# xaedes/ros_gpu_depthmap_fusion

Measured on AMD Instinct MI355X. Metric: Mpoints/s end-to-end depth→fused voxel grid @1/2/4/8 GPU; % HBM roofline, higher is better.
Workload: dtype f32; 1 GPU; C2: 640x480 u16 depth (dense frames), launch defaults (F=4 thr 0.3, crop/voxel -10..30/-20..20/-1..1.5, cells 0.1/0.1/0.12, voxelize average, lifetime 10); a step = a batch of 8 frames through one launch chain (every frame's points, voxel means and grid); cameras_per_gpu=1, steps=1630, warmup=5, prime=8, grid_cells=3360000, frames_in_flight=3, step_pmc_bytes=85523388, parallelism=single GPU

## Files before the change

### include/gdf.h

```cpp
#ifndef GDF_H_
#define GDF_H_

#include <stddef.h>
#include <stdint.h>

#ifdef __cplusplus
extern "C" {
#endif

#define GDF_VERSION_MAJOR 0
#define GDF_VERSION_MINOR 4

#define GDF_MAX_CAMERAS 16

enum gdf_status_code {
    GDF_OK = 0,
    GDF_ERR_ARG = -1,
    GDF_ERR_STATE = -2,
    GDF_ERR_HIP = -3,
    GDF_ERR_NOMEM = -4,
    GDF_ERR_CAPACITY = -5,
    GDF_ERR_TIME = -6,
    GDF_ERR_DEVICE = -7
};
// ... 129 lines not shown
    const float* points;
    const uint32_t* voxel_coords;
    uint32_t num_points;
    const float* voxelized;
    uint32_t num_voxelized;
    const uint8_t* occupancy;
    uint64_t num_cells;
} gdf_host_frame;
int gdf_download_frame(gdf_engine* engine, uint32_t what, gdf_host_frame* out);

int gdf_process_frame(gdf_engine* engine, const gdf_frame_params* params,
                      gdf_frame_result* out_result);

int gdf_get_graph_stats(gdf_engine* engine, uint64_t* captures, uint64_t* replays);
int gdf_last_sort_items(gdf_engine* engine, uint32_t* items, int* runs);

int gdf_mask_dilate(gdf_engine* engine, const uint32_t* in_mask_device, uint32_t* out_mask_device,
                    uint32_t width, uint32_t height, uint32_t filter_size, int as_written);
int gdf_transform_points(gdf_engine* engine, const float* in_points_device,
                         const uint32_t* mask_device, float* out_points_device, uint32_t num_items,
                         const float T[16]);

int gdf_next_frame_in_batch(gdf_engine* engine);
int gdf_get_batch_ranges(gdf_engine* engine, uint32_t* point_start, uint32_t* voxel_start,
                         uint32_t capacity, uint32_t* out_frames);
int gdf_download_batch_occupancy_grid(gdf_engine* engine, uint32_t frame, uint8_t* out,
                                      uint64_t capacity);

int gdf_export_occupancy_marks(gdf_engine* engine, uint32_t* device_bitmask, uint64_t words);
int gdf_import_occupancy_marks(gdf_engine* engine, const uint32_t* device_bitmasks,
// ... 85 lines not shown
```

### ros_gpu_depthmap_fusion_amd/csrc/gdf_device.hpp

```cpp
#pragma once

#include <hip/hip_runtime.h>
#include <stdint.h>

namespace gdf {

constexpr int kMaxCams = 16;
constexpr int kFrameThreads = 256;
constexpr int kArgCams = 8;
constexpr int kHalo = 8;
constexpr uint32_t kSegItems = 1024;
constexpr uint32_t kFusedPrefixSegs = 4096;
constexpr uint32_t kScanGroup = 64;
constexpr uint32_t kMaxScanGroups = 4096;
constexpr uint32_t kMaxGroupScanTiles = 65536;
constexpr uint32_t kSelSegs = 8;
constexpr uint32_t kSelThreads = 512;
constexpr int kSortThreads = 256;
constexpr int kSortGroup = 8;
constexpr int kHistReps = 16;
constexpr int kHistWords = kHistReps * 4 * 256;

__host__ __device__ constexpr uint32_t radix_passes(uint32_t bits) {
    return bits == 0 ? 1u : bits <= 25 ? (bits <= 9 ? 1u : (bits + 6) / 8) : (bits + 7) / 8;
}
__host__ __device__ constexpr bool radix_wide_last(uint32_t bits) {
    return bits >= 9 && bits <= 25 && bits % 8 == 1;
}
__host__ __device__ constexpr uint32_t radix_digit(uint32_t key, uint32_t p, uint32_t np) {
// ... 121 lines not shown
    uint32_t* grid_seq_out;
    uint32_t grid_seq;
    uint32_t nframes;
    uint32_t frame_shift;
    uint64_t mark_words;
    uint32_t* frame_pt_start;
    int32_t run_mode;
    uint32_t* wave_runs;
    uint32_t* run_keys;
    uint32_t* run_start;
    uint32_t* run_count;
    uint32_t* scan_total;
    uint32_t* run_total;
    uint32_t* grp_done;
    uint32_t* grp_tot;
    int32_t mask_packed;
    uint32_t nparts;
    uint64_t part_ncells;
    float4* part_pts;
    uint32_t* part_run_keys;
    uint32_t* part_run_starts;
    uint32_t* part_counts;
    uint32_t part_nseg;
    uint32_t seg_uniform;
    const Tuning* tune;
};
static_assert(sizeof(FrameArgs) <= 4096, "kernel arguments are limited to 4 KiB");

__device__ __forceinline__ float dot3(float ax, float ay, float az, float bx, float by, float bz) {
    return (ax * bx + ay * by) + az * bz;
// ... 52 lines not shown
```

### ros_gpu_depthmap_fusion_amd/csrc/gdf_engine.cpp

```cpp
#include <hip/hip_runtime.h>

#include <algorithm>
#include <cmath>
#include <cstdio>
#include <cstring>
#include <cstdlib>
#include <atomic>
#include <condition_variable>
#include <memory>
#include <mutex>
#include <string>
#include <thread>
#include <vector>

#include "gdf.h"
#include "gdf_kernels.hpp"

using namespace gdf;

namespace {
thread_local std::string g_last_error;
}

namespace gdf {
// ... 280 lines not shown
    DevBuf d_ka, d_kb, d_va, d_vb, d_sstatus, d_sgstatus, d_gstatus, d_ggstatus, d_vox;
    DevBuf d_gcnt, d_goff;
    DevBuf d_gfirst;
    DevBuf d_bigq, d_bigcnt;
    bool vox_valid = false;
    DevBuf d_markbits;
    uint32_t marks_gen = ~0u;
    uint32_t marks_frames = 0;
    DevBuf d_fstart, d_fvox;
    DevBuf d_snap_idx, d_snap_data, d_snap_cnt;
    bool snap_valid = false;
    uint32_t snap_blocks = 0, snap_frames = 0;
    DevBuf d_pcnt, d_poff;
    DevBuf d_xcnt, d_xoff, d_xrk, d_xrs;
    DevBuf d_grpdone, d_grptot;
    struct Pinned {
        void* p = nullptr;
        size_t bytes = 0;
        void* ensure(size_t need) {
            if (need <= bytes) return p;
            if (p) (void)hipHostFree(p);
            p = nullptr;
            bytes = 0;
            const size_t nb = std::max(need, bytes + bytes / 2);
            if (hipHostMalloc(&p, nb, hipHostMallocDefault) != hipSuccess) {
                p = nullptr;
                return nullptr;
            }
            bytes = nb;
            return p;
// ... 75 lines not shown
    PsBuf* collect = &psA;
    PsBuf* upload = &psB;

    std::vector<Cam> cams;
    uint32_t nframes = 1;
    uint32_t depth_total = 0;
    std::vector<CamDesc> halo;
    std::vector<Cam> halo_cams;
    std::vector<uint32_t> halo_tail;
    std::vector<CamTable> tables = std::vector<CamTable>(kMaxCams);
    std::vector<CamDesc> h_cams;
    uint32_t mask_blocks = 0;
    uint64_t index_end = 0;
    uint32_t last_sort_items = 0;
    bool last_sort_runs = false;
    uint32_t max_segw = 0;
    bool depth_uploaded = false;

    DevBuf d_new;
    uint32_t n_new = 0;
    std::vector<Hdr> new_hdrs;
    bool ps_filter_set = false;
    float ps_thr = 0.f;
    uint32_t ps_F = 0;

    DevBuf d_ring;
    uint64_t ring_cap = 0, ring_head = 0;
    std::vector<Hdr> hdrA, hdrB;
    uint32_t shard = 0, nshards = 1, shard_block = 1;
    uint64_t seq_counter = 0;
// ... 873 lines not shown
        q.d_runkeys.ensure((size_t)std::max<uint32_t>(q.n_total, 1) * 4);
        q.d_runstart.ensure(((size_t)q.n_total + 1) * 4);
        a.wave_runs = q.d_wruns.as<uint32_t>();
        a.run_keys = q.d_runkeys.as<uint32_t>();
        a.run_start = q.d_runstart.as<uint32_t>();
        a.run_count = q.d_misc.as<uint32_t>() + kRunCount;
        if (a.sel_tiles) a.run_total = q.d_misc.as<uint32_t>() + kRunTotal;
    }
    e->sl().runs_sel = a.run_mode && a.sel_tiles;
    a.vbits = e->sl().d_vbits.as<unsigned long long>();
    a.seg_counts = e->sl().d_tcounts.as<uint32_t>();
    a.seg_offsets = e->sl().d_toffsets.as<uint32_t>();
    a.fused_prefix = a.total_segs <= kFusedPrefixSegs ? 1 : 0;
    a.mask_packed = e->mask_packed ? 1 : 0;
    const uint32_t ngroups = (a.total_segs + kScanGroup - 1) / kScanGroup;
    if (!a.fused_prefix && e->group_scan && ngroups <= kMaxScanGroups) {
        Slot& q = e->sl();
        q.d_grpdone.ensure_zero((size_t)ngroups * 4, e->s());
        q.d_grptot.ensure((size_t)ngroups * 2 * 4);
        a.grp_done = q.d_grpdone.as<uint32_t>();
        a.grp_tot = q.d_grptot.as<uint32_t>();
    }
    {
        const uint32_t h = a.do_flying ? std::min<uint32_t>(a.F, kHalo) : 0u;
        const uint32_t cols = e->max_segw + 2 * h;
        a.band_rowb = ((cols * 2 + 15) / 16 + 1) * 16;
        a.band_lds = (2 * h + 1) * a.band_rowb + (kHalo + a.seg_threads * 2) * 4;
        a.hist_lds = (a.band_lds + 15) & ~15u;
        if (a.run_mode && a.key_hist) a.band_lds = a.hist_lds + 4 * 256 * 4;
    }
    if (e->debug) {
        e->sl().d_stage.ensure(std::max<size_t>({(size_t)e->sl().n_total, (size_t)e->index_end + sel, 1}));
        a.dbg = e->sl().d_stage.as<uint8_t>();
    }
    e->sl().dbg_count = e->sl().n_total;
    a.err = e->sl().d_misc.as<uint32_t>() + kErr;
    if (!e->halo_cams.empty() && a.do_flying && !e->cams.empty()) {
        for (size_t j = 0; j < e->halo_cams.size(); ++j) {
            const Cam* first = nullptr;
            for (const Cam& c : e->cams)
                if (c.frame == e->halo_cams[j].frame) { first = &c; break; }
            if (!first) continue;
            const uint64_t reach = (uint64_t)a.F * first->W + a.F;
            if (reach > e->halo_cams[j].n)
                fail(GDF_ERR_ARG, "halo camera shorter than F rows of the frame's first camera "
                                  "(reads would reach the camera before it)");
            if (e->halo_tail[j] < reach)
                fail(GDF_ERR_ARG, "halo depth map tail shorter than F rows + F pixels of the frame's first camera");
        }
    }
    a.nframes = e->nframes;
    a.frame_shift = e->nframes > 1 ? e->key_bits : 0u;
    a.mark_words = mark_words(e);
    e->sl().sel_frame = a.sel_tiles != 0;
    if (fused_voxel && compaction_marks && e->epart.nparts && e->emit_part && !a.sel_tiles &&
        a.total_segs && !e->debug) {
        FrameArgs t = a;
        t.run_mode = 1;
        t.key_hist = nullptr;
        t.fused_prefix = 0;
        t.grp_done = t.grp_tot = nullptr;
        if (emit_partition_kernels(t)) {
            Slot& q = e->sl();
            const uint32_t segs = std::max<uint32_t>(a.total_segs, 1);
            const uint32_t P = e->epart.nparts;
            q.d_tcounts.ensure((size_t)segs * 2 * P * 4);
            q.d_toffsets.ensure(seg_offsets_words(2 * P * segs) * 4);
            q.d_wruns.ensure((size_t)segs * 16 * 4);
            t.seg_counts = q.d_tcounts.as<uint32_t>();
            t.seg_offsets = q.d_toffsets.as<uint32_t>();
            t.wave_runs = q.d_wruns.as<uint32_t>();
            t.nparts = P;
            t.part_ncells = e->ncells;
            t.part_pts = reinterpret_cast<float4*>(e->epart.pts);
            t.part_run_keys = e->epart.run_keys;
            t.part_run_starts = e->epart.run_starts;
            t.part_counts = e->epart.counts;
            t.part_nseg = e->epart.nseg;
            a = t;
        }
    }
    e->sl().nframes = e->nframes;
    e->sl().snap_valid = false;
    if (e->nframes > 1) {
        e->sl().d_fstart.ensure((size_t)(e->nframes + 1) * 4);
        a.frame_pt_start = e->sl().d_fstart.as<uint32_t>();
    }
    return a;
}

void frame_launched(gdf_engine* e, bool fused_voxel, bool key_hist, bool runs = false) {
    e->sl().khist_pending = fused_voxel && key_hist;
    e->sl().runs_valid = fused_voxel && runs;
    e->sl().compacted = true;
    e->sl().coords_valid = fused_voxel;
    e->sl().marks_set = fused_voxel;
    e->sl().vox_valid = false;
}

void run_frame(gdf_engine* e, bool fused_voxel, bool compaction_marks = false) {
    e->sl().pf_valid = false;
    const FrameArgs a = frame_args(e, fused_voxel, compaction_marks);
// ... 1189 lines not shown
            e->last_sort_runs = runs;
            e->last_sort_items = runs ? e->sl().h_misc[e->sl().runs_sel ? kRunTotal : kRunCount]
                                      : res.num_points;
        }
        if (r) *r = res;
    });
}

int gdf_last_sort_items(gdf_engine* e, uint32_t* items, int* runs) {
    ENGINE_OR_FAIL(e);
    if (items) *items = e->last_sort_items;
    if (runs) *runs = e->last_sort_runs ? 1 : 0;
    return GDF_OK;
}

int gdf_mask_dilate(gdf_engine* e, const uint32_t* in, uint32_t* out, uint32_t W, uint32_t H,
                    uint32_t F, int as_written) {
    ENGINE_OR_FAIL(e);
    return guarded(e, [&] {
        if ((!in || !out) && (uint64_t)W * H) fail(GDF_ERR_ARG, "mask_dilate: null mask");
        if (in == out && (uint64_t)W * H) fail(GDF_ERR_ARG, "mask_dilate: in-place is not supported");
        if (F > kDilateMaxF) fail(GDF_ERR_ARG, "mask_dilate: filter size above 16");
        HIPCHK(launch_mask_dilate(in, out, W, H, F, as_written, e->s()));
    });
}

int gdf_transform_points(gdf_engine* e, const float* in, const uint32_t* mask, float* out,
                         uint32_t n, const float T[16]) {
    ENGINE_OR_FAIL(e);
    return guarded(e, [&] {
// ... 490 lines not shown
```

### ros_gpu_depthmap_fusion_amd/csrc/gdf_kernels.hip

```cpp
#include <atomic>
#include "gdf_kernels.hpp"

#if defined(__HIP_DEVICE_COMPILE__) && !defined(__gfx950__)
#error "gdf_kernels.hip targets gfx950 (CDNA4) only: its coherence hand-offs use gfx950 cache bits"
#endif
#include "gdf_voxsum.hpp"

#include <algorithm>

namespace gdf {

template <class T>
using gptr = __attribute__((address_space(1))) T*;
template <class T>
__device__ __forceinline__ gptr<T> G(T* p) {
    return (gptr<T>)p;
}

typedef float f4v __attribute__((ext_vector_type(4)));
__device__ __forceinline__ float4 gld4(const float4* p, uint64_t i) {
    const f4v v = ((gptr<const f4v>)p)[i];
    return make_float4(v.x, v.y, v.z, v.w);
}
__device__ __forceinline__ void gst4(float4* p, uint64_t i, const float4& w) {
// ... 686 lines not shown
__device__ __forceinline__ void group_partials_finish(const FrameArgs& a, uint32_t s,
                                                      const GroupPart& p, uint32_t* s_red) {
    const int lane = threadIdx.x & 63, wid = threadIdx.x >> 6;
    const uint32_t g = s / kScanGroup;
    const uint32_t ng = (a.total_segs + kScanGroup - 1) / kScanGroup;
    uint32_t sum = 0, rsum = 0;
#pragma unroll
    for (int q = 0; q < 4; ++q) {
        const bool in = threadIdx.x + (uint32_t)q * blockDim.x < g;
        sum += in ? p.v[q] : 0u;
        rsum += in ? p.w[q] : 0u;
    }
    for (uint32_t t = threadIdx.x + 4u * blockDim.x; t < g; t += blockDim.x) {
        sum += G(a.grp_tot)[t];
        if (a.run_mode) rsum += G(a.grp_tot)[ng + t];
    }
    for (int o = 32; o > 0; o >>= 1) {
        sum += __shfl_xor(sum, o, 64);
        rsum += __shfl_xor(rsum, o, 64);
    }
    if (lane == 0) {
        s_red[wid] = sum;
        s_red[16 + wid] = rsum;
    }
}

template <bool ROT45, uint32_t FT>
__global__ __launch_bounds__(1024) void k_mask(FrameArgs a) {
    __shared__ CamDesc s_cams[kMaxCams];
    __shared__ float s_yn[2 * kHalo + 1];
// ... 373 lines not shown
    uint32_t* s_hist = reinterpret_cast<uint32_t*>(reinterpret_cast<uint8_t*>(s_dyn) + a.hist_lds);
    const int lane = threadIdx.x & 63, wid = threadIdx.x >> 6;
    if (a.nparts)
        for (uint32_t j = threadIdx.x; j < 2u * NWORDS * kMaxParts; j += NT) (&s_pc[0][0][0])[j] = 0u;
    const uint32_t n = gridDim.x, q8 = n / 8, r8 = n % 8, xcd = blockIdx.x % 8;
    const uint32_t s = xcd * q8 + min(xcd, r8) + blockIdx.x / 8;
    uint32_t bits[PX], rkey[PX];
#pragma unroll
    for (int j = 0; j < PX; ++j) {
        bits[j] = 0u;
        rkey[j] = 0xFFFFFFFFu;
    }
    const uint32_t i = threadIdx.x;
    if (a.run_mode && a.key_hist)
        for (uint32_t j = threadIdx.x; j < radix_hist_span(a.npasses); j += NT) s_hist[j] = 0;
    {
        const gptr<const CamDesc> gcam = G(cam_table(a));
        SegGeo sg = seg_geo(gcam, a.ncams, s, a.seg_uniform);
        struct {
            const uint16_t* depth;
            const float *xn, *yn;
            uint32_t W, H;
        } c = {gcam[sg.k].depth, gcam[sg.k].xn, gcam[sg.k].yn, gcam[sg.k].W, gcam[sg.k].H};
#ifdef GDF_TRACE_GROUPS
        asm volatile("" ::"s"(c.depth), "s"(c.W));
        GDF_MSTAMP(1);
#endif
        const int h = 4;
        const uint32_t ca = sg.x0 >= (uint32_t)h ? sg.x0 - h : 0u;
        const uint32_t cb = min(c.W, sg.x0 + sg.len + h);
        const uint32_t nrows = 2 * h + 1;
        uint8_t* band = reinterpret_cast<uint8_t*>(s_dyn);
        float* s_xn = reinterpret_cast<float*>(band + (size_t)nrows * a.band_rowb) + kHalo;
        const bool wrap = sg.x0 == 0 && sg.y >= (uint32_t)h && c.W >= (uint32_t)h;
        typedef uint32_t u4v __attribute__((ext_vector_type(4)));
        const uintptr_t dbase = reinterpret_cast<uintptr_t>(c.depth);
        const uint32_t nch = a.band_rowb / 16;
        u4v v[QR][QC];
// ... 153 lines not shown
    __syncthreads();
#ifdef GDF_TRACE_GROUPS
    GDF_MSTAMP(5);
#endif
    if (wid == 0) {
        if (a.nparts) {
            if ((uint32_t)lane < 2u * a.nparts) {
                const uint32_t kind = lane / a.nparts, p = lane % a.nparts;
                uint32_t c = 0;
                for (int w = 0; w < NWORDS; ++w) c += s_pc[kind][w][p];
                G(a.seg_counts)[(size_t)lane * a.total_segs + s] = c;
            }
        } else if (lane == 0) {
            uint32_t tt = 0, r = 0;
            for (int w = 0; w < NWORDS; ++w) tt += s_cnt[w];
            publish_count(a.seg_counts + s, tt);
            if (a.run_mode) {
                for (int w = 0; w < NWORDS; ++w) r += s_rcnt[w];
                publish_count(a.seg_counts + a.total_segs + s, r);
            }
        }
    }
    if (a.run_mode && a.key_hist) {
        const gptr<uint32_t> rep = G(a.key_hist + (blockIdx.x % kHistReps) * 1024u);
        for (uint32_t j = threadIdx.x; j < radix_hist_span(a.npasses); j += NT)
            if (s_hist[j])
                __hip_atomic_fetch_add(rep + j, s_hist[j], __ATOMIC_RELAXED, __HIP_MEMORY_SCOPE_AGENT);
    }
    if (a.grid_seq_out && blockIdx.x == 0 && threadIdx.x == 0) *a.grid_seq_out = a.grid_seq;
    group_scan_tail(a, s);
#ifdef GDF_TRACE_GROUPS
    GDF_MSTAMP(6);
    if (threadIdx.x == 0 && blockIdx.x < kMaskTraceSlots) {
        unsigned long long* g = g_mtrace[blockIdx.x];
        g[0] = mw0;
        g[1] = wall_clock64();
        for (int k = 1; k < 7; ++k) g[k + 1] = mt[k] - mt[k - 1];
    }
#endif
}

template <int PX, int SEGW>
__global__ __launch_bounds__(SEGW / PX) void k_mask_px(FrameArgs a) {
    mask_px_body<PX, SEGW>(a);
}
// ... 416 lines not shown
        asm volatile("" : "+s"(vw[w]));
        any |= vw[w];
    }
    if (!__builtin_amdgcn_readfirstlane((uint32_t)(any | (any >> 32))) && s != nblk - 1) {
        if (!fps) return;
        const bool first_of_frame =
            s == seg0 && (k == 0 || !cams[k - 1].emit || cams[k - 1].frame != fr);
        if (!first_of_frame) return;
    }
    for (uint32_t j = threadIdx.x; j < (1u << kMarkCacheBits); j += NT) s_mark[j] = 0xFFFFFFFFu;
    const bool hist = a.key_hist && !a.run_mode;
    if (hist)
        for (uint32_t i = threadIdx.x; i < radix_hist_span(a.npasses); i += NT) s_hist[i] = 0;
    GroupPart gp{};
    if (!a.fused_prefix && a.grp_tot) gp = group_partials_issue(a, s);
    const uint32_t i = threadIdx.x;
    const uint32_t j = s - seg0;
    const uint32_t y = j / nchunk;
    const uint32_t x0 = (j - y * nchunk) * segw;
    const uint32_t len = min(segw, W - x0);
    uint64_t m[2];
    uint32_t dval[2] = {0u, 0u};
    float xnv[2] = {0.0f, 0.0f};
    uint16_t dl[2];
    float xl[2];
#pragma unroll
    for (int q = 0; q < 2; ++q) {
        m[q] = 0;
#pragma unroll
        for (int w = 0; w < NW; ++w)
// ... 3 lines not shown
        xl[q] = G(cxn)[x0 + ic];
    }
#pragma unroll
    for (int q = 0; q < 2; ++q) {
        const bool in = i + (uint32_t)NT * q < len;
        dval[q] = in ? dl[q] : 0u;
        xnv[q] = in ? xl[q] : 0.0f;
    }
    const float ynv = G(cyn)[y];
    uint32_t pc[NWORDS], rc[NWORDS];
#pragma unroll
    for (int w = 0; w < NWORDS; ++w) {
        pc[w] = (uint32_t)__popcll(vw[w]);
        rc[w] = 0u;
    }
    const uint32_t sbase = a.fused_prefix ? 0u : G(a.seg_offsets)[s];
    uint32_t rbase = 0;
    if (a.run_mode) {
        if (!a.fused_prefix)
            rbase = G(a.seg_offsets)[a.total_segs + s] -
                    (a.grp_tot ? 0u : G(a.seg_offsets)[a.total_segs]);
#pragma unroll
        for (int w = 0; w < NWORDS; ++w) rc[w] = G(a.wave_runs)[(size_t)s * 16 + w];
    }
    if (a.fused_prefix) prefix_partials(a, s, s_red);
    else if (a.grp_tot) group_partials_finish(a, s, gp, s_red);
    __syncthreads();
    uint32_t base = sbase;
    if (a.fused_prefix || a.grp_tot)
        for (int w = 0; w < NW; ++w) {
            base += s_red[w];
            rbase += s_red[16 + w];
        }
    uint32_t tot = 0, rtot = 0;
#pragma unroll
    for (int w = 0; w < NWORDS; ++w) {
        tot += pc[w];
        rtot += rc[w];
    }
    if (s == gridDim.x - 1 && threadIdx.x == 0) {
        *G(a.out_count) = base + tot;
        if (a.run_mode) {
            G(a.run_start)[rbase + rtot] = base + tot;
            *G(a.run_count) = rbase + rtot;
        }
    }
    if (a.frame_pt_start && threadIdx.x == 0) {
        const bool first_of_frame =
            s == seg0 && (k == 0 || !cams[k - 1].emit || cams[k - 1].frame != fr);
        if (first_of_frame) G(a.frame_pt_start)[fr] = base;
        if (s == gridDim.x - 1) G(a.frame_pt_start)[a.nframes] = base + tot;
    }
    const unsigned long long ltm = lanemask_lt();
    const f2v zz2 = f2((float)dval[0], (float)dval[1]) * f2(cams[k].scale, cams[k].scale);
    const f2v px2 = f2(xnv[0], xnv[1]) * zz2, py2 = f2(ynv, ynv) * zz2, pz2 = zz2;
    const f2v wx2 = mrow2(cams[k].Tw + 0, px2, py2, pz2), wy2 = mrow2(cams[k].Tw + 4, px2, py2, pz2);
    const f2v wz2 = mrow2(cams[k].Tw + 8, px2, py2, pz2), ww2 = mrow2(cams[k].Tw + 12, px2, py2, pz2);
    uint32_t key2[2] = {0xFFFFFFFFu, 0xFFFFFFFFu};
    if (a.do_voxel && (m[0] | m[1]))
        voxel_key2(wx2, wy2, wz2, a.vlo, a.vcs, a.vrcs, a.gmax, a.gs, key2[0], key2[1]);
// ... 299 lines not shown
                hipLaunchKernelGGL((k_mask_px<2, 256>), dim3(a.total_segs), dim3(128), lds, s, a);
            else if (km == reinterpret_cast<const void*>(&k_mask_px_o8<2, 256>))
                hipLaunchKernelGGL((k_mask_px_o8<2, 256>), dim3(a.total_segs), dim3(128), lds, s, a);
            else if (km == reinterpret_cast<const void*>(&k_mask_px<2, 640>))
                hipLaunchKernelGGL((k_mask_px<2, 640>), dim3(a.total_segs), dim3(320), lds, s, a);
            else if (km == reinterpret_cast<const void*>(&k_mask<true, 4>))
                hipLaunchKernelGGL((k_mask<true, 4>), dim3(a.total_segs), dim3(a.seg_threads), lds, s, a);
            else if (km == reinterpret_cast<const void*>(&k_mask<false, 4>))
                hipLaunchKernelGGL((k_mask<false, 4>), dim3(a.total_segs), dim3(a.seg_threads), lds, s, a);
            else if (a.rot45)
                hipLaunchKernelGGL((k_mask<true, 0>), dim3(a.total_segs), dim3(a.seg_threads), lds, s, a);
            else
                hipLaunchKernelGGL((k_mask<false, 0>), dim3(a.total_segs), dim3(a.seg_threads), lds, s, a);
            if ((e = hipGetLastError()) != hipSuccess) return e;
        }
        if (!a.fused_prefix && !a.grp_done) {
            HookScope hs(hook, GDF_KERNEL_SCAN);
            const uint32_t m = a.nparts ? 2u * a.nparts * a.total_segs
                                        : a.run_mode ? 2u * a.total_segs : a.total_segs;
            if ((e = launch_scan(a.seg_counts, m, a.seg_offsets, a.scan_total, nullptr, 1u, s)) != hipSuccess)
                return e;
        }
        HookScope hs(hook, GDF_KERNEL_EMIT);
        const void* ke = emit_kernel(a);
        if (ke == reinterpret_cast<const void*>(&k_emit_px2_parts<256>))
            hipLaunchKernelGGL(k_emit_px2_parts<256>, dim3(a.total_segs), dim3(128), 0, s, a);
        else if (ke == reinterpret_cast<const void*>(&k_emit_px2<256>))
            hipLaunchKernelGGL(k_emit_px2<256>, dim3(a.total_segs), dim3(128), 0, s, a);
        else if (ke == reinterpret_cast<const void*>(&k_emit_px2<640>))
            hipLaunchKernelGGL(k_emit_px2<640>, dim3(a.total_segs), dim3(320), 0, s, a);
        else
// ... 24 lines not shown
                           : reinterpret_cast<const void*>(&k_mask_px<2, 256>);
    if (T.mask_px2 >= 2 && a.do_flying && a.F == 4 && !a.rot45 && a.seg_threads == 640 && !a.dbg &&
        a.band_rowb <= 2 * 64 * 16 && a.total_segs >= kPx640MinSegs)
        return reinterpret_cast<const void*>(&k_mask_px<2, 640>);
    return frame_kernel(0, a.rot45, a.do_flying ? a.F : 0u);
}


bool emit_partition_kernels(const FrameArgs& a) {
    const void* km = mask_kernel(a);
    FrameArgs plain = a;
    plain.nparts = 0;
    return (km == reinterpret_cast<const void*>(&k_mask_px<2, 256>) ||
            km == reinterpret_cast<const void*>(&k_mask_px_o8<2, 256>)) &&
           emit_kernel(plain) == reinterpret_cast<const void*>(&k_emit_px2<256>);
}

const void* emit_kernel(const FrameArgs& a) {
    if (a.nparts) return reinterpret_cast<const void*>(&k_emit_px2_parts<256>);
    if (a.tune->emit_px2 && a.seg_threads == 256) return reinterpret_cast<const void*>(&k_emit_px2<256>);
    if (a.tune->emit_px2 && a.seg_threads == 640 && a.total_segs >= kPx640MinSegs)
        return reinterpret_cast<const void*>(&k_emit_px2<640>);
    return reinterpret_cast<const void*>(&k_emit);
}

const void* frame_kernel(int which, int rot45, uint32_t F) {
    if (which == 1) return reinterpret_cast<const void*>(&k_emit);
    if (which == 2) return reinterpret_cast<const void*>(&k_sel<8>);
    if (which == 4) return reinterpret_cast<const void*>(&k_sel<4>);
    if (which == 5) return reinterpret_cast<const void*>(&k_sel<16>);
// ... 2678 lines not shown
```

### ros_gpu_depthmap_fusion_amd/csrc/gdf_kernels.hpp

```cpp
#pragma once

#include "gdf.h"

__host__ __device__ inline uint32_t part_slice_words(uint32_t nparts, uint64_t ncells) {
    return (uint32_t)(((ncells + 31) / 32 + nparts - 1) / nparts);
}
#include "gdf_device.hpp"

#include <string>

namespace gdf {

void set_last_error(const std::string& msg);

struct LaunchHook {
    virtual void begin(int slot) = 0;
    virtual void end(int slot) = 0;
    virtual ~LaunchHook() = default;
};

struct VoxelParams {
    float vlo[3], vcs[3], gmax[3];
    uint32_t gs[3];
    float vrcs[3];
};

hipError_t launch_tables(uint32_t W, uint32_t H, float fx, float fy, float cx, float cy, float* xn,
                         float* yn, hipStream_t s);

hipError_t launch_frame(const FrameArgs& a, hipStream_t s, LaunchHook* hook = nullptr);
inline uint32_t scan_partials_offset(uint32_t segs) { return (segs + 63u) & ~63u; }
inline size_t seg_offsets_words(uint32_t segs) {
    return scan_partials_offset(segs) + (segs + 4095u) / 4096u + 1u;
}
const void* frame_kernel(int which, int rot45, uint32_t F = 0);
bool sel_key_lds_allowed(uint32_t bytes);
const void* mask_kernel(const FrameArgs& a);
const void* emit_kernel(const FrameArgs& a);
bool emit_partition_kernels(const FrameArgs& a);

hipError_t launch_ps_filter_insert(const float4* new_pts, uint32_t n, int do_filter, float thr,
                                   uint32_t F, float4* ring, uint64_t cap, uint64_t first,
                                   hipStream_t s, uint32_t src0 = 0, uint32_t cnt = 0xFFFFFFFFu);
hipError_t launch_gather_records(const void* rec, uint32_t n, uint32_t step, float4* out,
                                 hipStream_t s);

struct SnapArgs {
    uint32_t* idx;
    uint4* data;
    uint32_t* cnt;
};
void snap_dims(uint64_t ncells, uint32_t nblocks, uint32_t* waves, uint32_t* seg);
uint32_t fused_grid_blocks(uint64_t ncells, uint32_t wpt);
uint32_t batch_grid_blocks(uint64_t ncells);
// ... 147 lines not shown
```

### ros_gpu_depthmap_fusion_amd/gdf.py

```python
from __future__ import annotations

import ctypes as C
import os
from dataclasses import dataclass, field
from typing import Optional, Sequence

import numpy as np

_HERE = os.path.dirname(os.path.abspath(__file__))
LIB_PATH = os.path.join(_HERE, "lib", "libgdf.so")

GDF_OK = 0
STATUS_NAMES = {
    -1: "GDF_ERR_ARG", -2: "GDF_ERR_STATE", -3: "GDF_ERR_HIP", -4: "GDF_ERR_NOMEM",
    -5: "GDF_ERR_CAPACITY", -6: "GDF_ERR_TIME", -7: "GDF_ERR_DEVICE",
}

_f16 = C.c_float * 16
_f3 = C.c_float * 3


class RollbufferState(C.Structure):
    _fields_ = [(n, C.c_uint32) for n in (
        "num_points", "num_seqs", "selection_point_start", "selection_point_count",
# ... 91 lines not shown
    "gdf_insert_selected_point_sequence", "gdf_transform_point_sequence", "gdf_get_rollbuffer_state",
    "gdf_set_rollbuffer_shard", "gdf_get_rollbuffer_pieces",
    "gdf_upload_depthmaps", "gdf_convert_depthmaps", "gdf_filter_flying_pixels", "gdf_crop_points",
    "gdf_apply_point_mask", "gdf_compute_voxel_coords", "gdf_voxelize", "gdf_voxel_occupancy_grid",
    "gdf_get_point_count", "gdf_download_points", "gdf_download_voxel_coords",
    "gdf_download_voxelized_points", "gdf_download_occupancy_grid", "gdf_get_grid_size",
    "gdf_get_device_results", "gdf_process_frame", "gdf_export_occupancy_marks",
    "gdf_import_occupancy_marks", "gdf_take_occupancy_marks", "gdf_import_occupancy_marks_strided",
    "gdf_voxel_occupancy_grid_batch", "gdf_take_occupancy_marks_sparse", "gdf_union_occupancy_pairs",
    "gdf_set_profiling", "gdf_get_kernel_times", "gdf_set_debug", "gdf_debug_stage_masks", "gdf_debug_rollbuffer",
    "gdf_debug_historic_grid",
    "gdf_run_depth_stream", "gdf_run_host_stream", "gdf_run_depth_stream_batched",
    "gdf_run_depth_stream_alternating",
    "gdf_next_frame_in_batch", "gdf_get_batch_ranges", "gdf_download_batch_occupancy_grid",
    "gdf_mask_dilate", "gdf_transform_points", "gdf_add_halo_depthmap_device",
    "gdf_partition_points", "gdf_voxelize_points", "gdf_partition_runs", "gdf_voxelize_runs", "gdf_voxelize_runs_marked", "gdf_voxelize_runs_recv", "gdf_set_partition_marks", "gdf_set_emit_partition", "gdf_set_partition_segments", "gdf_last_sort_items", "gdf_get_stream",
    "gdf_get_graph_stats", "gdf_get_slot", "gdf_select_slot", "gdf_build_info", "gdf_get_tuning",
    "gdf_download_frame", "gdf_set_slot_streams",
    "gdf_fused_unique_id", "gdf_fused_create", "gdf_fused_destroy", "gdf_fused_halo_pixels",
    "gdf_fused_start", "gdf_fused_finish", "gdf_fused_run", "gdf_fused_local_create",
    "gdf_fused_local_destroy", "gdf_fused_create_local", "gdf_fused_info",
    "gdf_fused_set_rollbuffer_shard", "gdf_fused_local_check_round", "gdf_fused_local_check_arrival",
    "gdf_seg_create", "gdf_seg_destroy", "gdf_seg_set_stream", "gdf_seg_label_layers",
    "gdf_seg_label_engine_grid", "gdf_seg_get_counts", "gdf_seg_download_labels",
    "gdf_seg_download_num_labels", "gdf_seg_download_stats", "gdf_seg_download_connections",
    "gdf_seg_download_contours", "gdf_seg_merge_labels", "gdf_seg_get_device_results",
    "gdf_seg_create_objects",
]


ABI_VERSION = (0, 4)
# ... 71 lines not shown
        "gdf_next_frame_in_batch": (i32, [vp]),
        "gdf_mask_dilate": (i32, [vp, vp, vp, u32, u32, u32, i32]),
        "gdf_add_halo_depthmap_device": (i32, [vp, vp, u32, u32, u32, f, f, f, f, f, vp, vp]),
        "gdf_partition_points": (i32, [vp, u32, vp, vp, u32, vp]),
        "gdf_voxelize_points": (i32, [vp, vp, vp, u32, i32]),
        "gdf_partition_runs": (i32, [vp, u32, vp, vp, vp, u32, vp]),
        "gdf_set_emit_partition": (i32, [vp, u32, vp, vp, vp, u32, vp]),
        "gdf_voxelize_runs": (i32, [vp, vp, vp, vp, u32, vp, vp, i32]),
        "gdf_voxelize_runs_marked": (i32, [vp, vp, vp, vp, u32, vp, vp, i32, vp, u64]),
        "gdf_voxelize_runs_recv": (i32, [vp, vp, vp, vp, u32, vp, vp, i32, vp, u64, vp]),
        "gdf_set_partition_marks": (i32, [vp, i32]),
        "gdf_transform_points": (i32, [vp, vp, vp, vp, u32, vp]),
        "gdf_get_batch_ranges": (i32, [vp, vp, vp, u32, P(u32)]),
        "gdf_download_batch_occupancy_grid": (i32, [vp, u32, vp, u64]),
        "gdf_last_sort_items": (i32, [vp, P(u32), P(i32)]),
        "gdf_get_stream": (i32, [vp, P(vp)]),
        "gdf_get_graph_stats": (i32, [vp, P(u64), P(u64)]),
        "gdf_get_slot": (i32, [vp, P(i32)]),
        "gdf_select_slot": (i32, [vp, i32]),
        "gdf_build_info": (C.c_char_p, []),
        "gdf_get_tuning": (i32, [vp, C.c_char_p, u32]),
        "gdf_download_frame": (i32, [vp, u32, P(HostFrame)]),
        "gdf_set_slot_streams": (i32, [vp, vp, i32]),
        "gdf_fused_unique_id": (i32, [C.c_char_p, vp]),
        "gdf_fused_create": (i32, [vp, C.c_char_p, vp, i32, i32, P(StreamCamera), u32, P(vp)]),
        "gdf_fused_destroy": (i32, [vp]),
        "gdf_fused_halo_pixels": (i32, [vp, P(u32)]),
        "gdf_fused_start": (i32, [vp, vp, u32, P(FrameParams), P(i32)]),
        "gdf_fused_finish": (i32, [vp, i32, vp, P(u32)]),
        "gdf_fused_run": (i32, [vp, P(StreamCamera), P(FrameParams), u64, u64, u32, i32]),
# ... 559 lines not shown
    def graph_stats(self):
        c, r = C.c_uint64(0), C.c_uint64(0)
        self._check(self._lib.gdf_get_graph_stats(self._h, C.byref(c), C.byref(r)))
        return c.value, r.value

    def tuning(self) -> str:
        buf = C.create_string_buffer(4096)
        self._check(self._lib.gdf_get_tuning(self._h, buf, len(buf)))
        return buf.value.decode()

    def last_sort_items(self):
        n, r = C.c_uint32(0), C.c_int(0)
        self._check(self._lib.gdf_last_sort_items(self._h, C.byref(n), C.byref(r)))
        return n.value, bool(r.value)

    def processFramePrepared(self, p: FrameParams) -> FrameResult:
        r = FrameResult()
        self._check(self._lib.gdf_process_frame(self._h, C.byref(p), C.byref(r)))
        self._keep = []
        return r


SEG_CONTOURS, SEG_CONNECTIONS, SEG_ALL = 1, 2, 3


class Segmenter:

    def __init__(self, device: int = 0, lib_path: str = LIB_PATH):
        self._lib = load_library(lib_path)
        h = C.c_void_p()
# ... 86 lines not shown
```

Before: 35770 Mpoints/s.

## Replace group-scan tail with lazy double-buffered group totals in mask/emit kernels

Adds a lazy group-scan mode. Mask blocks atomically add their per-segment point and run counts into epoch-parity double-buffered group totals and re-arm the other buffer, instead of running the decoupled group_scan_tail. The emit kernel then sums the preceding group totals plus in-group counts directly to get its base offset, and bumps an epoch counter. The aim is to remove the tail-scan synchronisation and the seg_offsets dependency from the mask kernel, at the cost of more atomics and of emit blocks reading up to all prior group totals. It also adds a query API that reports the scan form used.

```diff
diff --git a/include/gdf.h b/include/gdf.h
--- a/include/gdf.h
+++ b/include/gdf.h
@@ -167,6 +167,7 @@
 
 int gdf_get_graph_stats(gdf_engine* engine, uint64_t* captures, uint64_t* replays);
 int gdf_last_sort_items(gdf_engine* engine, uint32_t* items, int* runs);
+int gdf_last_compaction(gdf_engine* engine, uint32_t* segments, int* scan_form);
 
 int gdf_mask_dilate(gdf_engine* engine, const uint32_t* in_mask_device, uint32_t* out_mask_device,
                     uint32_t width, uint32_t height, uint32_t filter_size, int as_written);
diff --git a/ros_gpu_depthmap_fusion_amd/csrc/gdf_device.hpp b/ros_gpu_depthmap_fusion_amd/csrc/gdf_device.hpp
--- a/ros_gpu_depthmap_fusion_amd/csrc/gdf_device.hpp
+++ b/ros_gpu_depthmap_fusion_amd/csrc/gdf_device.hpp
@@ -13,6 +13,8 @@
 constexpr uint32_t kFusedPrefixSegs = 4096;
 constexpr uint32_t kScanGroup = 64;
 constexpr uint32_t kMaxScanGroups = 4096;
+constexpr uint32_t kLazyHdr = 2;
+static_assert(kMaxScanGroups <= kFusedPrefixSegs, "a group-scan launch has a block per total");
 constexpr uint32_t kMaxGroupScanTiles = 65536;
 constexpr uint32_t kSelSegs = 8;
 constexpr uint32_t kSelThreads = 512;
@@ -164,6 +166,7 @@
     uint32_t* run_total;
     uint32_t* grp_done;
     uint32_t* grp_tot;
+    uint32_t* grp_lazy;
     int32_t mask_packed;
     uint32_t nparts;
     uint64_t part_ncells;
diff --git a/ros_gpu_depthmap_fusion_amd/csrc/gdf_engine.cpp b/ros_gpu_depthmap_fusion_amd/csrc/gdf_engine.cpp
--- a/ros_gpu_depthmap_fusion_amd/csrc/gdf_engine.cpp
+++ b/ros_gpu_depthmap_fusion_amd/csrc/gdf_engine.cpp
@@ -318,6 +318,7 @@
     DevBuf d_pcnt, d_poff;
     DevBuf d_xcnt, d_xoff, d_xrk, d_xrs;
     DevBuf d_grpdone, d_grptot;
+    DevBuf d_grplazy;
     struct Pinned {
         void* p = nullptr;
         size_t bytes = 0;
@@ -423,6 +424,8 @@
     uint64_t index_end = 0;
     uint32_t last_sort_items = 0;
     bool last_sort_runs = false;
+    uint32_t last_segs = 0;
+    int last_scan_form = 0;
     uint32_t max_segw = 0;
     bool depth_uploaded = false;
 
@@ -1326,13 +1329,6 @@
     a.fused_prefix = a.total_segs <= kFusedPrefixSegs ? 1 : 0;
     a.mask_packed = e->mask_packed ? 1 : 0;
     const uint32_t ngroups = (a.total_segs + kScanGroup - 1) / kScanGroup;
-    if (!a.fused_prefix && e->group_scan && ngroups <= kMaxScanGroups) {
-        Slot& q = e->sl();
-        q.d_grpdone.ensure_zero((size_t)ngroups * 4, e->s());
-        q.d_grptot.ensure((size_t)ngroups * 2 * 4);
-        a.grp_done = q.d_grpdone.as<uint32_t>();
-        a.grp_tot = q.d_grptot.as<uint32_t>();
-    }
     {
         const uint32_t h = a.do_flying ? std::min<uint32_t>(a.F, kHalo) : 0u;
         const uint32_t cols = e->max_segw + 2 * h;
@@ -1347,6 +1343,18 @@
     }
     e->sl().dbg_count = e->sl().n_total;
     a.err = e->sl().d_misc.as<uint32_t>() + kErr;
+    if (!a.fused_prefix && e->group_scan && ngroups <= kMaxScanGroups) {
+        Slot& q = e->sl();
+        if (lazy_group_scan_kernels(a)) {
+            q.d_grplazy.ensure_zero((size_t)(kLazyHdr + 4 * kMaxScanGroups) * 4, e->s());
+            a.grp_lazy = q.d_grplazy.as<uint32_t>();
+        } else {
+            q.d_grpdone.ensure_zero((size_t)ngroups * 4, e->s());
+            q.d_grptot.ensure((size_t)ngroups * 2 * 4);
+            a.grp_done = q.d_grpdone.as<uint32_t>();
+            a.grp_tot = q.d_grptot.as<uint32_t>();
+        }
+    }
     if (!e->halo_cams.empty() && a.do_flying && !e->cams.empty()) {
         for (size_t j = 0; j < e->halo_cams.size(); ++j) {
             const Cam* first = nullptr;
@@ -1372,6 +1380,7 @@
         t.key_hist = nullptr;
         t.fused_prefix = 0;
         t.grp_done = t.grp_tot = nullptr;
+        t.grp_lazy = nullptr;
         if (emit_partition_kernels(t)) {
             Slot& q = e->sl();
             const uint32_t segs = std::max<uint32_t>(a.total_segs, 1);
@@ -1398,6 +1407,8 @@
         e->sl().d_fstart.ensure((size_t)(e->nframes + 1) * 4);
         a.frame_pt_start = e->sl().d_fstart.as<uint32_t>();
     }
+    e->last_segs = a.total_segs;
+    e->last_scan_form = a.fused_prefix ? 0 : a.grp_lazy ? 3 : a.grp_done ? 2 : 1;
     return a;
 }
 
@@ -2617,6 +2628,13 @@
     return GDF_OK;
 }
 
+int gdf_last_compaction(gdf_engine* e, uint32_t* segments, int* scan_form) {
+    ENGINE_OR_FAIL(e);
+    if (segments) *segments = e->last_segs;
+    if (scan_form) *scan_form = e->last_scan_form;
+    return GDF_OK;
+}
+
 int gdf_mask_dilate(gdf_engine* e, const uint32_t* in, uint32_t* out, uint32_t W, uint32_t H,
                     uint32_t F, int as_written) {
     ENGINE_OR_FAIL(e);
diff --git a/ros_gpu_depthmap_fusion_amd/csrc/gdf_kernels.hip b/ros_gpu_depthmap_fusion_amd/csrc/gdf_kernels.hip
--- a/ros_gpu_depthmap_fusion_amd/csrc/gdf_kernels.hip
+++ b/ros_gpu_depthmap_fusion_amd/csrc/gdf_kernels.hip
@@ -724,6 +724,77 @@
     for (uint32_t t = threadIdx.x + 4u * blockDim.x; t < g; t += blockDim.x) {
         sum += G(a.grp_tot)[t];
         if (a.run_mode) rsum += G(a.grp_tot)[ng + t];
+    }
+    for (int o = 32; o > 0; o >>= 1) {
+        sum += __shfl_xor(sum, o, 64);
+        rsum += __shfl_xor(rsum, o, 64);
+    }
+    if (lane == 0) {
+        s_red[wid] = sum;
+        s_red[16 + wid] = rsum;
+    }
+}
+
+__device__ __forceinline__ void lazy_publish(const FrameArgs& a, uint32_t s, uint32_t epoch,
+                                             uint32_t pts, uint32_t runs) {
+    G(a.seg_counts)[s] = pts;
+    if (a.run_mode) G(a.seg_counts)[a.total_segs + s] = runs;
+    const gptr<uint32_t> tot =
+        G(a.grp_lazy) + kLazyHdr + (epoch & 1u) * 2u * kMaxScanGroups + 2u * (s / kScanGroup);
+    if (pts) __hip_atomic_fetch_add(tot, pts, __ATOMIC_RELAXED, __HIP_MEMORY_SCOPE_AGENT);
+    if (runs) __hip_atomic_fetch_add(tot + 1, runs, __ATOMIC_RELAXED, __HIP_MEMORY_SCOPE_AGENT);
+}
+__device__ __forceinline__ void lazy_rearm(const FrameArgs& a, uint32_t s, uint32_t epoch) {
+    typedef uint32_t u2v __attribute__((ext_vector_type(2)));
+    if (s >= kMaxScanGroups) return;
+    const gptr<u2v> other = (gptr<u2v>)(a.grp_lazy + kLazyHdr) + ((epoch & 1u) ^ 1u) * kMaxScanGroups;
+    u2v z;
+    z.x = z.y = 0u;
+    other[s] = z;
+}
+
+struct LazyPart {
+    uint32_t v[4][2][2];
+    uint32_t c[2];
+};
+typedef uint32_t lazy_u2v __attribute__((ext_vector_type(2)));
+__device__ __forceinline__ LazyPart lazy_partials_issue(const FrameArgs& a, uint32_t s) {
+    LazyPart p;
+    const uint32_t g = s / kScanGroup;
+    const uint32_t last = g ? g - 1u : 0u;
+    const gptr<const lazy_u2v> set0 = (gptr<const lazy_u2v>)(a.grp_lazy + kLazyHdr);
+#pragma unroll
+    for (int q = 0; q < 4; ++q) {
+        const uint32_t t = min(threadIdx.x + (uint32_t)q * blockDim.x, last);
+#pragma unroll
+        for (int e = 0; e < 2; ++e) {
+            const lazy_u2v x = set0[e * kMaxScanGroups + t];
+            p.v[q][e][0] = x.x;
+            p.v[q][e][1] = x.y;
+        }
+    }
+    const uint32_t c = min(g * kScanGroup + threadIdx.x, s);
+    p.c[0] = G(a.seg_counts)[c];
+    p.c[1] = a.run_mode ? G(a.seg_counts)[a.total_segs + c] : 0u;
+    return p;
+}
+__device__ __forceinline__ void lazy_partials_finish(const FrameArgs& a, uint32_t s,
+                                                     const LazyPart& p, uint32_t* s_red) {
+    const int lane = threadIdx.x & 63, wid = threadIdx.x >> 6;
+    const uint32_t g = s / kScanGroup;
+    const bool own = g * kScanGroup + threadIdx.x < s;
+    uint32_t sum = own ? p.c[0] : 0u, rsum = own ? p.c[1] : 0u;
+#pragma unroll
+    for (int q = 0; q < 4; ++q) {
+        const bool in = threadIdx.x + (uint32_t)q * blockDim.x < g;
+        sum += in ? p.v[q][0][0] + p.v[q][1][0] : 0u;
+        rsum += in ? p.v[q][0][1] + p.v[q][1][1] : 0u;
+    }
+    const gptr<const lazy_u2v> set0 = (gptr<const lazy_u2v>)(a.grp_lazy + kLazyHdr);
+    for (uint32_t t = threadIdx.x + 4u * blockDim.x; t < g; t += blockDim.x) {
+        const lazy_u2v x = set0[t], y = set0[kMaxScanGroups + t];
+        sum += x.x + y.x;
+        rsum += x.y + y.y;
     }
     for (int o = 32; o > 0; o >>= 1) {
         sum += __shfl_xor(sum, o, 64);
@@ -1127,6 +1198,7 @@
     const uint32_t i = threadIdx.x;
     if (a.run_mode && a.key_hist)
         for (uint32_t j = threadIdx.x; j < radix_hist_span(a.npasses); j += NT) s_hist[j] = 0;
+    uint32_t lazy_epoch = 0;
     {
         const gptr<const CamDesc> gcam = G(cam_table(a));
         SegGeo sg = seg_geo(gcam, a.ncams, s, a.seg_uniform);
@@ -1135,6 +1207,7 @@
             const float *xn, *yn;
             uint32_t W, H;
         } c = {gcam[sg.k].depth, gcam[sg.k].xn, gcam[sg.k].yn, gcam[sg.k].W, gcam[sg.k].H};
+        if (a.grp_lazy) lazy_epoch = G(a.grp_lazy)[0];
 #ifdef GDF_TRACE_GROUPS
         asm volatile("" ::"s"(c.depth), "s"(c.W));
         GDF_MSTAMP(1);
@@ -1318,12 +1391,17 @@
         } else if (lane == 0) {
             uint32_t tt = 0, r = 0;
             for (int w = 0; w < NWORDS; ++w) tt += s_cnt[w];
-            publish_count(a.seg_counts + s, tt);
-            if (a.run_mode) {
+            if (a.run_mode)
                 for (int w = 0; w < NWORDS; ++w) r += s_rcnt[w];
-                publish_count(a.seg_counts + a.total_segs + s, r);
-            }
-        }
+            if (a.grp_lazy) {
+                lazy_publish(a, s, lazy_epoch, tt, r);
+            } else {
+                publish_count(a.seg_counts + s, tt);
+                if (a.run_mode) publish_count(a.seg_counts + a.total_segs + s, r);
+            }
+        }
+    } else if (a.grp_lazy && threadIdx.x == 64) {
+        lazy_rearm(a, s, lazy_epoch);
     }
     if (a.run_mode && a.key_hist) {
         const gptr<uint32_t> rep = G(a.key_hist + (blockIdx.x % kHistReps) * 1024u);
@@ -1332,7 +1410,7 @@
                 __hip_atomic_fetch_add(rep + j, s_hist[j], __ATOMIC_RELAXED, __HIP_MEMORY_SCOPE_AGENT);
     }
     if (a.grid_seq_out && blockIdx.x == 0 && threadIdx.x == 0) *a.grid_seq_out = a.grid_seq;
-    group_scan_tail(a, s);
+    if (!a.grp_lazy) group_scan_tail(a, s);
 #ifdef GDF_TRACE_GROUPS
     GDF_MSTAMP(6);
     if (threadIdx.x == 0 && blockIdx.x < kMaskTraceSlots) {
@@ -1779,6 +1857,8 @@
         for (uint32_t i = threadIdx.x; i < radix_hist_span(a.npasses); i += NT) s_hist[i] = 0;
     GroupPart gp{};
     if (!a.fused_prefix && a.grp_tot) gp = group_partials_issue(a, s);
+    LazyPart lp{};
+    if (a.grp_lazy) lp = lazy_partials_issue(a, s);
     const uint32_t i = threadIdx.x;
     const uint32_t j = s - seg0;
     const uint32_t y = j / nchunk;
@@ -1812,20 +1892,22 @@
         pc[w] = (uint32_t)__popcll(vw[w]);
         rc[w] = 0u;
     }
-    const uint32_t sbase = a.fused_prefix ? 0u : G(a.seg_offsets)[s];
+    const bool offs = !a.fused_prefix && !a.grp_lazy;
+    const uint32_t sbase = offs ? G(a.seg_offsets)[s] : 0u;
     uint32_t rbase = 0;
     if (a.run_mode) {
-        if (!a.fused_prefix)
+        if (offs)
             rbase = G(a.seg_offsets)[a.total_segs + s] -
                     (a.grp_tot ? 0u : G(a.seg_offsets)[a.total_segs]);
 #pragma unroll
         for (int w = 0; w < NWORDS; ++w) rc[w] = G(a.wave_runs)[(size_t)s * 16 + w];
     }
     if (a.fused_prefix) prefix_partials(a, s, s_red);
+    else if (a.grp_lazy) lazy_partials_finish(a, s, lp, s_red);
     else if (a.grp_tot) group_partials_finish(a, s, gp, s_red);
     __syncthreads();
     uint32_t base = sbase;
-    if (a.fused_prefix || a.grp_tot)
+    if (a.fused_prefix || a.grp_tot || a.grp_lazy)
         for (int w = 0; w < NW; ++w) {
             base += s_red[w];
             rbase += s_red[16 + w];
@@ -1842,6 +1924,8 @@
             G(a.run_start)[rbase + rtot] = base + tot;
             *G(a.run_count) = rbase + rtot;
         }
+        if (a.grp_lazy)
+            __hip_atomic_fetch_add(G(a.grp_lazy), 1u, __ATOMIC_RELAXED, __HIP_MEMORY_SCOPE_AGENT);
     }
     if (a.frame_pt_start && threadIdx.x == 0) {
         const bool first_of_frame =
@@ -2171,7 +2255,7 @@
                 hipLaunchKernelGGL((k_mask<false, 0>), dim3(a.total_segs), dim3(a.seg_threads), lds, s, a);
             if ((e = hipGetLastError()) != hipSuccess) return e;
         }
-        if (!a.fused_prefix && !a.grp_done) {
+        if (!a.fused_prefix && !a.grp_done && !a.grp_lazy) {
             HookScope hs(hook, GDF_KERNEL_SCAN);
             const uint32_t m = a.nparts ? 2u * a.nparts * a.total_segs
                                         : a.run_mode ? 2u * a.total_segs : a.total_segs;
@@ -2226,6 +2310,17 @@
     return (km == reinterpret_cast<const void*>(&k_mask_px<2, 256>) ||
             km == reinterpret_cast<const void*>(&k_mask_px_o8<2, 256>)) &&
            emit_kernel(plain) == reinterpret_cast<const void*>(&k_emit_px2<256>);
+}
+
+bool lazy_group_scan_kernels(const FrameArgs& a) {
+    const void* km = mask_kernel(a);
+    const void* ke = emit_kernel(a);
+    return !a.nparts &&
+           (km == reinterpret_cast<const void*>(&k_mask_px<2, 256>) ||
+            km == reinterpret_cast<const void*>(&k_mask_px_o8<2, 256>) ||
+            km == reinterpret_cast<const void*>(&k_mask_px<2, 640>)) &&
+           (ke == reinterpret_cast<const void*>(&k_emit_px2<256>) ||
+            ke == reinterpret_cast<const void*>(&k_emit_px2<640>));
 }
 
 const void* emit_kernel(const FrameArgs& a) {
diff --git a/ros_gpu_depthmap_fusion_amd/csrc/gdf_kernels.hpp b/ros_gpu_depthmap_fusion_amd/csrc/gdf_kernels.hpp
--- a/ros_gpu_depthmap_fusion_amd/csrc/gdf_kernels.hpp
+++ b/ros_gpu_depthmap_fusion_amd/csrc/gdf_kernels.hpp
@@ -38,6 +38,7 @@
 const void* mask_kernel(const FrameArgs& a);
 const void* emit_kernel(const FrameArgs& a);
 bool emit_partition_kernels(const FrameArgs& a);
+bool lazy_group_scan_kernels(const FrameArgs& a);
 
 hipError_t launch_ps_filter_insert(const float4* new_pts, uint32_t n, int do_filter, float thr,
                                    uint32_t F, float4* ring, uint64_t cap, uint64_t first,
diff --git a/ros_gpu_depthmap_fusion_amd/gdf.py b/ros_gpu_depthmap_fusion_amd/gdf.py
--- a/ros_gpu_depthmap_fusion_amd/gdf.py
+++ b/ros_gpu_depthmap_fusion_amd/gdf.py
@@ -129,7 +129,7 @@
     "gdf_run_depth_stream_alternating",
     "gdf_next_frame_in_batch", "gdf_get_batch_ranges", "gdf_download_batch_occupancy_grid",
     "gdf_mask_dilate", "gdf_transform_points", "gdf_add_halo_depthmap_device",
-    "gdf_partition_points", "gdf_voxelize_points", "gdf_partition_runs", "gdf_voxelize_runs", "gdf_voxelize_runs_marked", "gdf_voxelize_runs_recv", "gdf_set_partition_marks", "gdf_set_emit_partition", "gdf_set_partition_segments", "gdf_last_sort_items", "gdf_get_stream",
+    "gdf_partition_points", "gdf_voxelize_points", "gdf_partition_runs", "gdf_voxelize_runs", "gdf_voxelize_runs_marked", "gdf_voxelize_runs_recv", "gdf_set_partition_marks", "gdf_set_emit_partition", "gdf_set_partition_segments", "gdf_last_sort_items", "gdf_last_compaction", "gdf_get_stream",
     "gdf_get_graph_stats", "gdf_get_slot", "gdf_select_slot", "gdf_build_info", "gdf_get_tuning",
     "gdf_download_frame", "gdf_set_slot_streams",
     "gdf_fused_unique_id", "gdf_fused_create", "gdf_fused_destroy", "gdf_fused_halo_pixels",
@@ -231,6 +231,7 @@
         "gdf_get_batch_ranges": (i32, [vp, vp, vp, u32, P(u32)]),
         "gdf_download_batch_occupancy_grid": (i32, [vp, u32, vp, u64]),
         "gdf_last_sort_items": (i32, [vp, P(u32), P(i32)]),
+        "gdf_last_compaction": (i32, [vp, P(u32), P(i32)]),
         "gdf_get_stream": (i32, [vp, P(vp)]),
         "gdf_get_graph_stats": (i32, [vp, P(u64), P(u64)]),
         "gdf_get_slot": (i32, [vp, P(i32)]),
@@ -820,6 +821,11 @@
         self._check(self._lib.gdf_last_sort_items(self._h, C.byref(n), C.byref(r)))
         return n.value, bool(r.value)
 
+    def last_compaction(self):
+        n, f = C.c_uint32(0), C.c_int(0)
+        self._check(self._lib.gdf_last_compaction(self._h, C.byref(n), C.byref(f)))
+        return n.value, f.value
+
     def processFramePrepared(self, p: FrameParams) -> FrameResult:
         r = FrameResult()
         self._check(self._lib.gdf_process_frame(self._h, C.byref(p), C.byref(r)))
```

New measurement: 36380 Mpoints/s (median of 6 runs). 1.7% higher.
